# jianzongwu/DiffSensei

Measured on NVIDIA H100. Metric: unet_denoise_steps_per_sec_1024sq_bs4, higher is better.
Workload: dtype bf16

## Files before the change

### diffsensei_b200/csrc/attn_wgmma.cu

```cuda
#include <cstdlib>

#include "ds_common.cuh"
#include "ds_host.h"
#include "ip_mask.cuh"
#include "wgmma.cuh"

namespace ds {

constexpr int kQTile = 128;
constexpr int kKTile = 64;
constexpr int kHd = 64;
constexpr int kRing = 4;
constexpr int kAttnThreads = 384;
constexpr int kQBytes = kQTile * kHd * 2;
constexpr int kKVBytes = kKTile * kHd * 2;
constexpr int kAttnSmemBytes = kQBytes + kRing * 2 * kKVBytes + 1024  + 256 ;
constexpr float kLog2e = 1.4426950408889634f;

struct AttnParams {
  __nv_bfloat16* out;
  int Nq, ldo;
  int n_keys[2];
  int k_col0, v_col0;
  float scale_log2;
  const float* bbox;
  int num_ips, tokens_per_ip, num_dummy, Hd, Wd;
  float ip_scale;
};

__device__ __forceinline__ float ex2(float x) {
  float y;
  asm("ex2.approx.ftz.f32 %0, %1;" : "=f"(y) : "f"(x));
  return y;
}

__global__ void __launch_bounds__(kAttnThreads, 1)
attn_wgmma_kernel(const __grid_constant__ CUtensorMap tmQ, const __grid_constant__ CUtensorMap tmK0,
                  const __grid_constant__ CUtensorMap tmK1, const AttnParams p) {
  extern __shared__ uint8_t smem_raw[];
  const uint32_t raw_addr = smem_u32(smem_raw);
  uint8_t* smem = smem_raw + ((1024u - (raw_addr & 1023u)) & 1023u);
  uint8_t* sQ = smem;
  uint8_t* sRing = sQ + kQBytes;
  uint64_t* q_bar = reinterpret_cast<uint64_t*>(sRing + kRing * 2 * kKVBytes);
  uint64_t* full_bar = q_bar + 1;
  uint64_t* empty_bar = full_bar + kRing;

  const int warp = threadIdx.x >> 5, lane = threadIdx.x & 31;
  const int q0 = blockIdx.x * kQTile, head = blockIdx.y, b = blockIdx.z;
  const int tiles0 = (p.n_keys[0] + kKTile - 1) / kKTile;
  const int tiles1 = (p.n_keys[1] + kKTile - 1) / kKTile;

  if (warp == 0 && lane == 0) {
    tma_prefetch_desc(&tmQ);
    tma_prefetch_desc(&tmK0);
    if (tiles1 > 0) tma_prefetch_desc(&tmK1);
    mbar_init(q_bar, 1);
    for (int i = 0; i < kRing; ++i) {
      mbar_init(&full_bar[i], 1);
      mbar_init(&empty_bar[i], 256);
    }
    fence_mbar_init();
  }
  pdl_launch_dependents();
  __syncthreads();
  pdl_wait();

  if (warp < 4) {
    if (warp == 0 && lane == 0) {
      mbar_arrive_expect_tx(q_bar, kQBytes);
      tma_load_3d(sQ, &tmQ, q_bar, head * kHd, q0, b);
      int stage = 0;
      uint32_t phase = 0;
      for (int t = 0; t < tiles0 + tiles1; ++t) {
        const bool second = t >= tiles0;
        const CUtensorMap* m = second ? &tmK1 : &tmK0;
        const int key0 = (second ? t - tiles0 : t) * kKTile;
        mbar_wait(&empty_bar[stage], phase ^ 1);
        mbar_arrive_expect_tx(&full_bar[stage], 2 * kKVBytes);
        uint8_t* sK = sRing + stage * 2 * kKVBytes;
        tma_load_3d(sK, m, &full_bar[stage], p.k_col0 + head * kHd, key0, b);
        tma_load_3d(sK + kKVBytes, m, &full_bar[stage], p.v_col0 + head * kHd, key0, b);
        if (++stage == kRing) {
          stage = 0;
          phase ^= 1;
        }
      }
    }
    return;
  }

  const int ct = threadIdx.x - 128;
  const int wg = ct >> 7;
  const int r0 = (ct >> 5) * 16 + (lane >> 2);
  const int cq = 2 * (lane & 3);
  uint32_t ip_bits[2] = {0u, 0u};
  if (tiles1 > 0) {
    const float* bb = p.bbox + static_cast<size_t>(b) * p.num_ips * 4;
#pragma unroll
    for (int h = 0; h < 2; ++h) {
      const int n = q0 + r0 + 8 * h;
      if (n < p.Nq) ip_bits[h] = ip_inside_bits(bb, p.num_ips, n, p.Hd, p.Wd);
    }
  }
  const uint32_t q_addr = smem_u32(sQ) + wg * 64 * 128;
  mbar_wait(q_bar, 0);

  float o[32], res[32];
  float m_run[2], l_run[2];
  int stage = 0;
  uint32_t phase = 0;
  for (int set = 0; set < (tiles1 > 0 ? 2 : 1); ++set) {
    const int n_tiles = set ? tiles1 : tiles0;
    const int nk = set ? p.n_keys[1] : p.n_keys[0];
#pragma unroll
    for (int i = 0; i < 32; ++i) o[i] = 0.f;
    m_run[0] = m_run[1] = -INFINITY;
    l_run[0] = l_run[1] = 0.f;
    for (int t = 0; t < n_tiles; ++t) {
      mbar_wait(&full_bar[stage], phase);
      const uint32_t k_addr = smem_u32(sRing + stage * 2 * kKVBytes);
      const uint32_t v_addr = k_addr + kKVBytes;
      float s[32];
      wgmma_fence();
#pragma unroll
      for (int k = 0; k < kHd / 16; ++k)
        wgmma_m64n64_ss(s, make_wgmma_desc(q_addr + k * 32, 1024, 16), make_wgmma_desc(k_addr + k * 32, 1024, 16),
                        k != 0);
      wgmma_commit();
      wgmma_wait<0>();
      fence_regs<32>(s);

      const int key0 = t * kKTile;
      float mx[2] = {-INFINITY, -INFINITY};
#pragma unroll
      for (int j = 0; j < 8; ++j) {
#pragma unroll
        for (int e = 0; e < 4; ++e) {
          const int key = key0 + j * 8 + cq + (e & 1);
          const int h = e >> 1;
          float v = s[4 * j + e] * p.scale_log2;
          if (set == 1 && !ip_key_open(ip_bits[h], key, p.tokens_per_ip, p.num_dummy)) v -= 10000.0f * kLog2e;
          if (key >= nk) v = -INFINITY;
          s[4 * j + e] = v;
          mx[h] = fmaxf(mx[h], v);
        }
      }
      float corr[2];
#pragma unroll
      for (int h = 0; h < 2; ++h) {
        mx[h] = fmaxf(mx[h], __shfl_xor_sync(0xffffffffu, mx[h], 1));
        mx[h] = fmaxf(mx[h], __shfl_xor_sync(0xffffffffu, mx[h], 2));
        const float m_new = fmaxf(m_run[h], mx[h]);
        corr[h] = ex2(m_run[h] - m_new);
        m_run[h] = m_new;
        l_run[h] *= corr[h];
      }
      uint32_t pa[4][4];
#pragma unroll
      for (int j = 0; j < 8; ++j) {
#pragma unroll
        for (int h = 0; h < 2; ++h) {
          const float p0 = ex2(s[4 * j + 2 * h] - m_run[h]);
          const float p1 = ex2(s[4 * j + 2 * h + 1] - m_run[h]);
          l_run[h] += p0 + p1;
          pa[j >> 1][(j & 1) * 2 + h] = pack_bf16(p0, p1);
        }
      }
#pragma unroll
      for (int j = 0; j < 8; ++j) {
        o[4 * j + 0] *= corr[0];
        o[4 * j + 1] *= corr[0];
        o[4 * j + 2] *= corr[1];
        o[4 * j + 3] *= corr[1];
      }
      wgmma_fence();
#pragma unroll
      for (int kk = 0; kk < kKTile / 16; ++kk)
        wgmma_m64n64_rs_tb(o, pa[kk], make_wgmma_desc(v_addr + kk * 2048, 1024, 1024), 1);
      wgmma_commit();
      wgmma_wait<0>();
      fence_regs<32>(o);
      mbar_arrive(&empty_bar[stage]);
      if (++stage == kRing) {
        stage = 0;
        phase ^= 1;
      }
    }
#pragma unroll
    for (int h = 0; h < 2; ++h) {
      l_run[h] += __shfl_xor_sync(0xffffffffu, l_run[h], 1);
      l_run[h] += __shfl_xor_sync(0xffffffffu, l_run[h], 2);
    }
    const float w = set ? p.ip_scale : 1.0f;
    const float inv[2] = {w / l_run[0], w / l_run[1]};
#pragma unroll
    for (int i = 0; i < 32; ++i) {
      const float v = o[i] * inv[(i >> 1) & 1];
      res[i] = set ? res[i] + v : v;
    }
  }

#pragma unroll
  for (int h = 0; h < 2; ++h) {
    const int n = q0 + r0 + 8 * h;
    if (n >= p.Nq) continue;
    __nv_bfloat16* orow = p.out + (static_cast<size_t>(b) * p.Nq + n) * p.ldo + head * kHd + cq;
#pragma unroll
    for (int j = 0; j < 8; ++j)
      *reinterpret_cast<uint32_t*>(orow + j * 8) = pack_bf16(res[4 * j + 2 * h], res[4 * j + 2 * h + 1]);
  }
}

static bool make_tok_map(CUtensorMap* m, const void* base, int cols, int ld, int tokens, int batch, int box_rows) {
  const uint64_t dims[3] = {static_cast<uint64_t>(cols), static_cast<uint64_t>(tokens), static_cast<uint64_t>(batch)};
  const uint64_t strides[2] = {static_cast<uint64_t>(ld) * 2, static_cast<uint64_t>(tokens) * ld * 2};
  const uint32_t box[3] = {kHd, static_cast<uint32_t>(box_rows), 1};
  return encode_tmap_bf16(m, base, 3, dims, strides, box, nullptr);
}

static int launch_attn(const CUtensorMap& tmQ, const CUtensorMap& tmK0, const CUtensorMap& tmK1, const AttnParams& p,
                       int B, int heads, cudaStream_t st) {
  static bool attr_set[kMaxDevices] = {};
  bool& set = attr_set[device_slot()];
  if (!set) {
    DS_CUDA_OK(cudaFuncSetAttribute(attn_wgmma_kernel, cudaFuncAttributeMaxDynamicSharedMemorySize, kAttnSmemBytes));
    set = true;
  }
  cudaLaunchConfig_t cfg = {};
  cfg.gridDim = dim3((p.Nq + kQTile - 1) / kQTile, heads, B);
  cfg.blockDim = dim3(kAttnThreads);
  cfg.dynamicSmemBytes = kAttnSmemBytes;
  cfg.stream = st;
  cudaLaunchAttribute attr[1];
  pdl_attr(&attr[0]);
  cfg.attrs = attr;
  cfg.numAttrs = 1;
  DS_CUDA_OK(cudaLaunchKernelEx(&cfg, attn_wgmma_kernel, tmQ, tmK0, tmK1, p));
  DS_LAUNCH_OK("attn_wgmma_kernel");
  return DS_OK;
}

static int launch_flash(const void* q, int ldq, int q_cols, const void* kv, int ldkv, int kv_cols, int k_col0,
                        int v_col0, void* out, int ldo, int B, int Nq, int Nkv, int heads, float scale, cudaStream_t st) {
  DeviceInfo dev;
  if (!get_device(&dev)) return DS_ERR_CUDA;
  CUtensorMap tmQ, tmK;
  if (!make_tok_map(&tmQ, q, q_cols, ldq, Nq, B, kQTile)) return DS_ERR_CUDA;
  if (!make_tok_map(&tmK, kv, kv_cols, ldkv, Nkv, B, kKTile)) return DS_ERR_CUDA;
  AttnParams p{};
  p.out = static_cast<__nv_bfloat16*>(out);
  p.Nq = Nq;
  p.ldo = ldo;
  p.n_keys[0] = Nkv;
  p.n_keys[1] = 0;
  p.k_col0 = k_col0;
  p.v_col0 = v_col0;
  p.scale_log2 = scale * kLog2e;
  return launch_attn(tmQ, tmK, tmK, p, B, heads, st);
}

}

using namespace ds;

extern "C" int ds_attention_self(const void* qkv, void* out, int B, int N, int heads, void* stream) {
  DS_REQUIRE(qkv && out, "ds_attention_self: NULL pointer");
  DS_REQUIRE(B > 0 && N > 0 && heads > 0, "ds_attention_self: bad shape");
  DS_REQUIRE((reinterpret_cast<uintptr_t>(qkv) & 15) == 0 && (reinterpret_cast<uintptr_t>(out) & 15) == 0,
             "ds_attention_self: pointers must be 16-byte aligned");
  const int C = heads * kHd;
  return launch_flash(qkv, 3 * C, 3 * C, qkv, 3 * C, 3 * C, C, 2 * C, out, C, B, N, N, heads, 0.125f,
                      static_cast<cudaStream_t>(stream));
}

extern "C" int ds_resampler_attn(const void* q, const void* kv, void* out, int Bc, int nq, int n_kv, int heads,
                                 void* stream) {
  DS_REQUIRE(q && kv && out, "ds_resampler_attn: NULL pointer");
  DS_REQUIRE(Bc > 0 && nq > 0 && n_kv > 0 && heads > 0, "ds_resampler_attn: bad shape");
  DS_REQUIRE((reinterpret_cast<uintptr_t>(q) & 15) == 0 && (reinterpret_cast<uintptr_t>(kv) & 15) == 0 &&
                 (reinterpret_cast<uintptr_t>(out) & 15) == 0,
             "ds_resampler_attn: pointers must be 16-byte aligned");
  const int C = heads * kHd;
  return launch_flash(q, C, C, kv, 2 * C, 2 * C, 0, C, out, C, Bc, nq, n_kv, heads, 0.125f,
                      static_cast<cudaStream_t>(stream));
}

extern "C" int ds_attention_cross_ip(const ds_cross_ip_args* a, void* stream) {
  DS_REQUIRE(a != nullptr, "ds_attention_cross_ip: args is NULL");
  DS_REQUIRE(a->q && a->kv_text && a->kv_ip && a->bbox && a->out, "ds_attention_cross_ip: NULL pointer");
  DS_REQUIRE(a->B > 0 && a->N > 0 && a->heads > 0, "ds_attention_cross_ip: bad shape");
  DS_REQUIRE(a->n_text > 0 && a->n_ip > 0, "ds_attention_cross_ip: n_text and n_ip must be positive");
  DS_REQUIRE(a->num_ips > 0 && a->num_ips <= kMaxIps && a->tokens_per_ip > 0 && a->num_dummy >= 0 &&
                 a->num_dummy + a->num_ips * a->tokens_per_ip == a->n_ip,
             "ds_attention_cross_ip: n_ip (%d) != num_dummy (%d) + num_ips (%d) * tokens_per_ip (%d)", a->n_ip,
             a->num_dummy, a->num_ips, a->tokens_per_ip);
  DS_REQUIRE((reinterpret_cast<uintptr_t>(a->q) & 15) == 0 && (reinterpret_cast<uintptr_t>(a->kv_text) & 15) == 0 &&
                 (reinterpret_cast<uintptr_t>(a->kv_ip) & 15) == 0 && (reinterpret_cast<uintptr_t>(a->out) & 15) == 0,
             "ds_attention_cross_ip: pointers must be 16-byte aligned");
  int Hd, Wd;
  if (!derive_hw(a->N, a->aspect_ratio, &Hd, &Wd)) {
    set_error("ds_attention_cross_ip: cannot factor N=%d for aspect_ratio=%f", a->N, a->aspect_ratio);
    return DS_ERR_INVALID;
  }
  DeviceInfo dev;
  if (!get_device(&dev)) return DS_ERR_CUDA;
  const int C = a->heads * kHd;
  CUtensorMap tmQ, tmT, tmI;
  if (!make_tok_map(&tmQ, a->q, C, C, a->N, a->B, kQTile)) return DS_ERR_CUDA;
  if (!make_tok_map(&tmT, a->kv_text, 2 * C, 2 * C, a->n_text, a->B, kKTile)) return DS_ERR_CUDA;
  if (!make_tok_map(&tmI, a->kv_ip, 2 * C, 2 * C, a->n_ip, a->B, kKTile)) return DS_ERR_CUDA;
  AttnParams p{};
  p.out = static_cast<__nv_bfloat16*>(a->out);
  p.Nq = a->N;
  p.ldo = C;
  p.n_keys[0] = a->n_text;
  p.n_keys[1] = a->n_ip;
  p.k_col0 = 0;
  p.v_col0 = C;
  p.scale_log2 = 0.125f * kLog2e;
  p.bbox = a->bbox;
  p.num_ips = a->num_ips;
  p.tokens_per_ip = a->tokens_per_ip;
  p.num_dummy = a->num_dummy;
  p.Hd = Hd;
  p.Wd = Wd;
  p.ip_scale = a->ip_scale;
  return launch_attn(tmQ, tmT, tmI, p, a->B, a->heads, static_cast<cudaStream_t>(stream));
}
```

### diffsensei_b200/csrc/ip_mask.cuh

```cuda
#pragma once
#include <math.h>
#include <stdint.h>

namespace ds {

constexpr int kMaxIps = 16;

inline bool derive_hw(int N, double aspect_ratio, int* Hd, int* Wd) {
  if (N <= 0 || !(aspect_ratio > 0.0)) return false;
  long long width = static_cast<long long>(pow(static_cast<double>(N) / aspect_ratio, 0.5));
  if (width < 1) return false;
  long long height = N / width;
  while (width * height != N) {
    if (width * height < N)
      width += 1;
    else
      width -= 1;
    if (width < 1 || width > N) return false;
    height = N / width;
  }
  *Hd = static_cast<int>(height);
  *Wd = static_cast<int>(width);
  return true;
}

__device__ __forceinline__ float linspace01(int i, int steps) {
  if (steps <= 1) return 0.0f;
  const float step = __fdiv_rn(1.0f, static_cast<float>(steps - 1));
  return (i < steps / 2) ? __fmul_rn(step, static_cast<float>(i))
                         : __fmaf_rn(-step, static_cast<float>(steps - 1 - i), 1.0f);
}

__device__ __forceinline__ uint32_t ip_inside_bits(const float* __restrict__ bbox, int num_ips, int n, int Hd, int Wd) {
  const int yi = n / Wd, xi = n - yi * Wd;
  const float x = linspace01(xi, Wd), y = linspace01(yi, Hd);
  uint32_t bits = 0;
  for (int i = 0; i < num_ips; ++i) {
    const float x1 = bbox[4 * i], y1 = bbox[4 * i + 1], x2 = bbox[4 * i + 2], y2 = bbox[4 * i + 3];
    if (x >= x1 && x <= x2 && y >= y1 && y <= y2) bits |= 1u << i;
  }
  return bits;
}

__device__ __forceinline__ bool ip_key_open(uint32_t bits, int key, int tokens_per_ip, int num_dummy) {
  if (key < num_dummy) return bits == 0;
  return (bits >> ((key - num_dummy) / tokens_per_ip)) & 1u;
}

}
```

Baseline: 5.116.

## Pipeline QK/PV wgmma, add persistent resident-KV cross-attention kernel, rebalance registers

Restructures the attention loop so the next tile's QK^T wgmma is issued while the current tile's PV wgmma runs, overlapping softmax with tensor-core work. Adds setmaxnreg to shift registers from the producer warpgroup to the consumers. Adds a persistent cross-attention kernel that keeps the short text+IP KV resident in shared memory across query tiles and double-buffers Q loads. It also precomputes the IP mask as a 64-bit key bitmap and skips masking on full unmasked tiles. The pipelining raises register pressure and adds more complex synchronisation.

```diff
diff --git a/diffsensei_b200/csrc/attn_wgmma.cu b/diffsensei_b200/csrc/attn_wgmma.cu
--- a/diffsensei_b200/csrc/attn_wgmma.cu
+++ b/diffsensei_b200/csrc/attn_wgmma.cu
@@ -14,8 +14,13 @@
 constexpr int kAttnThreads = 384;
 constexpr int kQBytes = kQTile * kHd * 2;
 constexpr int kKVBytes = kKTile * kHd * 2;
-constexpr int kAttnSmemBytes = kQBytes + kRing * 2 * kKVBytes + 1024  + 256 ;
+constexpr int kStreamSmemBytes = kQBytes + kRing * 2 * kKVBytes + 1024  + 256 ;
+constexpr int kResidentTiles = 4;
+constexpr int kQBufs = 2;
+constexpr int kCrossSmemBytes = kResidentTiles * 2 * kKVBytes + kQBufs * kQBytes + 1024 + 256;
 constexpr float kLog2e = 1.4426950408889634f;
+constexpr int kProducerRegs = 40;
+constexpr int kConsumerRegs = 232;
 
 struct AttnParams {
   __nv_bfloat16* out;
@@ -26,6 +31,7 @@
   const float* bbox;
   int num_ips, tokens_per_ip, num_dummy, Hd, Wd;
   float ip_scale;
+  int heads, q_tiles, items;
 };
 
 __device__ __forceinline__ float ex2(float x) {
@@ -34,9 +40,205 @@
   return y;
 }
 
+struct SetMask {
+  int nk;
+  bool ip;
+  uint32_t ip_bits[2];
+  int tokens_per_ip, num_dummy;
+};
+
+__device__ __forceinline__ void issue_qk(float (&s)[32], uint32_t q_addr, uint32_t k_addr) {
+#pragma unroll
+  for (int k = 0; k < kHd / 16; ++k)
+    wgmma_m64n64_ss(s, make_wgmma_desc(q_addr + k * 32, 1024, 16), make_wgmma_desc(k_addr + k * 32, 1024, 16), k != 0);
+}
+
+__device__ __forceinline__ void issue_pv(float (&o)[32], const uint32_t (&pa)[4][4], uint32_t v_addr) {
+#pragma unroll
+  for (int kk = 0; kk < kKTile / 16; ++kk)
+    wgmma_m64n64_rs_tb(o, pa[kk], make_wgmma_desc(v_addr + kk * 2048, 1024, 1024), 1);
+}
+
+__device__ __forceinline__ void fence_operands(float (&o)[32], uint32_t (&pa)[4][4]) {
+  fence_regs<32>(o);
+#pragma unroll
+  for (int kk = 0; kk < 4; ++kk)
+#pragma unroll
+    for (int i = 0; i < 4; ++i) asm volatile("" : "+r"(pa[kk][i])::"memory");
+}
+
+template <bool kMasked>
+__device__ __forceinline__ void softmax_step(const float (&s)[32], int key0, const SetMask& mk,
+                                             const uint64_t (&open)[2], float scale_log2, int cq, float (&m_run)[2],
+                                             float (&l_run)[2], float (&corr)[2], uint32_t (&pa)[4][4]) {
+  float x[32];
+  float mx[2] = {-INFINITY, -INFINITY};
+#pragma unroll
+  for (int j = 0; j < 8; ++j) {
+#pragma unroll
+    for (int e = 0; e < 4; ++e) {
+      const int key = key0 + j * 8 + cq + (e & 1);
+      const int h = e >> 1;
+      float v = s[4 * j + e] * scale_log2;
+      if (kMasked) {
+        if (mk.ip && !((open[h] >> (j * 8 + (e & 1))) & 1u)) v -= 10000.0f * kLog2e;
+        if (key >= mk.nk) v = -INFINITY;
+      }
+      x[4 * j + e] = v;
+      mx[h] = fmaxf(mx[h], v);
+    }
+  }
+#pragma unroll
+  for (int h = 0; h < 2; ++h) {
+    mx[h] = fmaxf(mx[h], __shfl_xor_sync(0xffffffffu, mx[h], 1));
+    mx[h] = fmaxf(mx[h], __shfl_xor_sync(0xffffffffu, mx[h], 2));
+    const float m_new = fmaxf(m_run[h], mx[h]);
+    corr[h] = ex2(m_run[h] - m_new);
+    m_run[h] = m_new;
+    l_run[h] *= corr[h];
+  }
+#pragma unroll
+  for (int j = 0; j < 8; ++j) {
+#pragma unroll
+    for (int h = 0; h < 2; ++h) {
+      const float p0 = ex2(x[4 * j + 2 * h] - m_run[h]);
+      const float p1 = ex2(x[4 * j + 2 * h + 1] - m_run[h]);
+      l_run[h] += p0 + p1;
+      pa[j >> 1][(j & 1) * 2 + h] = pack_bf16(p0, p1);
+    }
+  }
+}
+
+__device__ __forceinline__ void softmax_tile(const float (&s)[32], int key0, const SetMask& mk, float scale_log2, int cq,
+                                             float (&m_run)[2], float (&l_run)[2], float (&corr)[2],
+                                             uint32_t (&pa)[4][4]) {
+  uint64_t open[2] = {0ull, 0ull};
+  if (mk.ip) {
+#pragma unroll
+    for (int h = 0; h < 2; ++h)
+      open[h] = ip_open_keys64(mk.ip_bits[h], key0, mk.tokens_per_ip, mk.num_dummy) >> cq;
+  }
+  if (mk.ip || key0 + kKTile > mk.nk)
+    softmax_step<true>(s, key0, mk, open, scale_log2, cq, m_run, l_run, corr, pa);
+  else
+    softmax_step<false>(s, key0, mk, open, scale_log2, cq, m_run, l_run, corr, pa);
+}
+
+template <class TileAddr, class Release>
+__device__ __forceinline__ void attend_set(float (&o)[32], float (&l_run)[2], uint32_t q_addr, int n_tiles,
+                                           const SetMask& mk, float scale_log2, int cq, TileAddr tile_addr,
+                                           Release release) {
+  float m_run[2] = {-INFINITY, -INFINITY};
+  l_run[0] = l_run[1] = 0.f;
+#pragma unroll
+  for (int i = 0; i < 32; ++i) o[i] = 0.f;
+  float s[32], corr[2];
+  uint32_t pa[4][4], pb[4][4];
+  uint32_t k_addr = tile_addr(0);
+  wgmma_fence();
+  issue_qk(s, q_addr, k_addr);
+  wgmma_commit();
+  wgmma_wait<0>();
+  fence_regs<32>(s);
+  softmax_tile(s, 0, mk, scale_log2, cq, m_run, l_run, corr, pa);
+
+  auto step = [&](int t, uint32_t(&cur)[4][4], uint32_t(&next)[4][4]) {
+    const uint32_t k_next = tile_addr(t + 1);
+    fence_operands(o, cur);
+    wgmma_fence();
+    issue_qk(s, q_addr, k_next);
+    wgmma_commit();
+    issue_pv(o, cur, k_addr + kKVBytes);
+    wgmma_commit();
+    wgmma_wait<1>();
+    fence_regs<32>(s);
+    softmax_tile(s, (t + 1) * kKTile, mk, scale_log2, cq, m_run, l_run, corr, next);
+    wgmma_wait<0>();
+    fence_regs<32>(o);
+    release(t);
+#pragma unroll
+    for (int j = 0; j < 8; ++j) {
+      o[4 * j + 0] *= corr[0];
+      o[4 * j + 1] *= corr[0];
+      o[4 * j + 2] *= corr[1];
+      o[4 * j + 3] *= corr[1];
+    }
+    k_addr = k_next;
+  };
+  auto last = [&](int t, uint32_t(&cur)[4][4]) {
+    fence_operands(o, cur);
+    wgmma_fence();
+    issue_pv(o, cur, k_addr + kKVBytes);
+    wgmma_commit();
+    wgmma_wait<0>();
+    fence_regs<32>(o);
+    release(t);
+  };
+  for (int t = 0;; t += 2) {
+    if (t + 1 == n_tiles) {
+      last(t, pa);
+      break;
+    }
+    step(t, pa, pb);
+    if (t + 2 == n_tiles) {
+      last(t + 1, pb);
+      break;
+    }
+    step(t + 1, pb, pa);
+  }
+}
+
+__device__ __forceinline__ void normalise_into(float (&res)[32], const float (&o)[32], float (&l_run)[2], float w,
+                                               bool accumulate) {
+#pragma unroll
+  for (int h = 0; h < 2; ++h) {
+    l_run[h] += __shfl_xor_sync(0xffffffffu, l_run[h], 1);
+    l_run[h] += __shfl_xor_sync(0xffffffffu, l_run[h], 2);
+  }
+  const float inv[2] = {w / l_run[0], w / l_run[1]};
+#pragma unroll
+  for (int i = 0; i < 32; ++i) {
+    const float v = o[i] * inv[(i >> 1) & 1];
+    res[i] = accumulate ? res[i] + v : v;
+  }
+}
+
+__device__ __forceinline__ void store_rows(const AttnParams& p, const float (&res)[32], int b, int head, int row0,
+                                           int cq) {
+#pragma unroll
+  for (int h = 0; h < 2; ++h) {
+    const int n = row0 + 8 * h;
+    if (n >= p.Nq) continue;
+    __nv_bfloat16* orow = p.out + (static_cast<size_t>(b) * p.Nq + n) * p.ldo + head * kHd + cq;
+#pragma unroll
+    for (int j = 0; j < 8; ++j)
+      *reinterpret_cast<uint32_t*>(orow + j * 8) = pack_bf16(res[4 * j + 2 * h], res[4 * j + 2 * h + 1]);
+  }
+}
+
+__device__ __forceinline__ void ip_row_bits(const AttnParams& p, int b, int row0, uint32_t (&bits)[2]) {
+  const float* bb = p.bbox + static_cast<size_t>(b) * p.num_ips * 4;
+#pragma unroll
+  for (int h = 0; h < 2; ++h) {
+    const int n = row0 + 8 * h;
+    bits[h] = n < p.Nq ? ip_inside_bits(bb, p.num_ips, n, p.Hd, p.Wd) : 0u;
+  }
+}
+
+__device__ __forceinline__ SetMask set_mask(const AttnParams& p, int set, const uint32_t (&bits)[2]) {
+  SetMask mk;
+  mk.nk = set ? p.n_keys[1] : p.n_keys[0];
+  mk.ip = set == 1;
+  mk.ip_bits[0] = bits[0];
+  mk.ip_bits[1] = bits[1];
+  mk.tokens_per_ip = p.tokens_per_ip;
+  mk.num_dummy = p.num_dummy;
+  return mk;
+}
+
 __global__ void __launch_bounds__(kAttnThreads, 1)
-attn_wgmma_kernel(const __grid_constant__ CUtensorMap tmQ, const __grid_constant__ CUtensorMap tmK0,
-                  const __grid_constant__ CUtensorMap tmK1, const AttnParams p) {
+attn_stream_kernel(const __grid_constant__ CUtensorMap tmQ, const __grid_constant__ CUtensorMap tmK0,
+                   const __grid_constant__ CUtensorMap tmK1, const AttnParams p) {
   extern __shared__ uint8_t smem_raw[];
   const uint32_t raw_addr = smem_u32(smem_raw);
   uint8_t* smem = smem_raw + ((1024u - (raw_addr & 1023u)) & 1023u);
@@ -67,6 +269,7 @@
   pdl_wait();
 
   if (warp < 4) {
+    setmaxnreg_dec<kProducerRegs>();
     if (warp == 0 && lane == 0) {
       mbar_arrive_expect_tx(q_bar, kQBytes);
       tma_load_3d(sQ, &tmQ, q_bar, head * kHd, q0, b);
@@ -90,125 +293,142 @@
     return;
   }
 
+  setmaxnreg_inc<kConsumerRegs>();
   const int ct = threadIdx.x - 128;
   const int wg = ct >> 7;
   const int r0 = (ct >> 5) * 16 + (lane >> 2);
   const int cq = 2 * (lane & 3);
   uint32_t ip_bits[2] = {0u, 0u};
-  if (tiles1 > 0) {
-    const float* bb = p.bbox + static_cast<size_t>(b) * p.num_ips * 4;
-#pragma unroll
-    for (int h = 0; h < 2; ++h) {
-      const int n = q0 + r0 + 8 * h;
-      if (n < p.Nq) ip_bits[h] = ip_inside_bits(bb, p.num_ips, n, p.Hd, p.Wd);
-    }
-  }
+  if (tiles1 > 0) ip_row_bits(p, b, q0 + r0, ip_bits);
   const uint32_t q_addr = smem_u32(sQ) + wg * 64 * 128;
+  const uint32_t ring_addr = smem_u32(sRing);
   mbar_wait(q_bar, 0);
 
-  float o[32], res[32];
-  float m_run[2], l_run[2];
+  float o[32], res[32], l_run[2];
   int stage = 0;
   uint32_t phase = 0;
+  auto tile_addr = [&](int) {
+    mbar_wait(&full_bar[stage], phase);
+    const uint32_t a = ring_addr + stage * 2 * kKVBytes;
+    if (++stage == kRing) {
+      stage = 0;
+      phase ^= 1;
+    }
+    return a;
+  };
+  int rstage = 0;
+  auto release = [&](int) {
+    mbar_arrive(&empty_bar[rstage]);
+    if (++rstage == kRing) rstage = 0;
+  };
   for (int set = 0; set < (tiles1 > 0 ? 2 : 1); ++set) {
-    const int n_tiles = set ? tiles1 : tiles0;
-    const int nk = set ? p.n_keys[1] : p.n_keys[0];
-#pragma unroll
-    for (int i = 0; i < 32; ++i) o[i] = 0.f;
-    m_run[0] = m_run[1] = -INFINITY;
-    l_run[0] = l_run[1] = 0.f;
-    for (int t = 0; t < n_tiles; ++t) {
-      mbar_wait(&full_bar[stage], phase);
-      const uint32_t k_addr = smem_u32(sRing + stage * 2 * kKVBytes);
-      const uint32_t v_addr = k_addr + kKVBytes;
-      float s[32];
-      wgmma_fence();
-#pragma unroll
-      for (int k = 0; k < kHd / 16; ++k)
-        wgmma_m64n64_ss(s, make_wgmma_desc(q_addr + k * 32, 1024, 16), make_wgmma_desc(k_addr + k * 32, 1024, 16),
-                        k != 0);
-      wgmma_commit();
-      wgmma_wait<0>();
-      fence_regs<32>(s);
-
-      const int key0 = t * kKTile;
-      float mx[2] = {-INFINITY, -INFINITY};
-#pragma unroll
-      for (int j = 0; j < 8; ++j) {
-#pragma unroll
-        for (int e = 0; e < 4; ++e) {
-          const int key = key0 + j * 8 + cq + (e & 1);
-          const int h = e >> 1;
-          float v = s[4 * j + e] * p.scale_log2;
-          if (set == 1 && !ip_key_open(ip_bits[h], key, p.tokens_per_ip, p.num_dummy)) v -= 10000.0f * kLog2e;
-          if (key >= nk) v = -INFINITY;
-          s[4 * j + e] = v;
-          mx[h] = fmaxf(mx[h], v);
+    const SetMask mk = set_mask(p, set, ip_bits);
+    attend_set(o, l_run, q_addr, set ? tiles1 : tiles0, mk, p.scale_log2, cq, tile_addr, release);
+    normalise_into(res, o, l_run, set ? p.ip_scale : 1.0f, set != 0);
+  }
+  store_rows(p, res, b, head, q0 + r0, cq);
+}
+
+__global__ void __launch_bounds__(kAttnThreads, 1)
+attn_cross_kernel(const __grid_constant__ CUtensorMap tmQ, const __grid_constant__ CUtensorMap tmK0,
+                  const __grid_constant__ CUtensorMap tmK1, const AttnParams p) {
+  extern __shared__ uint8_t smem_raw[];
+  const uint32_t raw_addr = smem_u32(smem_raw);
+  uint8_t* smem = smem_raw + ((1024u - (raw_addr & 1023u)) & 1023u);
+  uint8_t* sKV = smem;
+  uint8_t* sQ = sKV + kResidentTiles * 2 * kKVBytes;
+  uint64_t* kv_full = reinterpret_cast<uint64_t*>(sQ + kQBufs * kQBytes);
+  uint64_t* kv_empty = kv_full + 1;
+  uint64_t* q_full = kv_empty + 1;
+  uint64_t* q_empty = q_full + kQBufs;
+
+  const int warp = threadIdx.x >> 5, lane = threadIdx.x & 31;
+  const int tiles0 = (p.n_keys[0] + kKTile - 1) / kKTile;
+  const int tiles1 = (p.n_keys[1] + kKTile - 1) / kKTile;
+  const int item_lo = static_cast<int>(static_cast<long long>(blockIdx.x) * p.items / gridDim.x);
+  const int item_hi = static_cast<int>(static_cast<long long>(blockIdx.x + 1) * p.items / gridDim.x);
+
+  if (warp == 0 && lane == 0) {
+    tma_prefetch_desc(&tmQ);
+    tma_prefetch_desc(&tmK0);
+    tma_prefetch_desc(&tmK1);
+    mbar_init(kv_full, 1);
+    mbar_init(kv_empty, 256);
+    for (int i = 0; i < kQBufs; ++i) {
+      mbar_init(&q_full[i], 1);
+      mbar_init(&q_empty[i], 256);
+    }
+    fence_mbar_init();
+  }
+  pdl_launch_dependents();
+  __syncthreads();
+  pdl_wait();
+
+  if (warp < 4) {
+    setmaxnreg_dec<kProducerRegs>();
+    if (warp == 0 && lane == 0) {
+      int pair = -1;
+      uint32_t kv_phase = 0;
+      for (int item = item_lo, it = 0; item < item_hi; ++item, ++it) {
+        const int ip = item / p.q_tiles, qt = item - ip * p.q_tiles;
+        const int b = ip / p.heads, head = ip - b * p.heads;
+        if (ip != pair) {
+          pair = ip;
+          mbar_wait(kv_empty, kv_phase ^ 1);
+          kv_phase ^= 1;
+          mbar_arrive_expect_tx(kv_full, (tiles0 + tiles1) * 2 * kKVBytes);
+          for (int t = 0; t < tiles0 + tiles1; ++t) {
+            const bool second = t >= tiles0;
+            const CUtensorMap* m = second ? &tmK1 : &tmK0;
+            const int key0 = (second ? t - tiles0 : t) * kKTile;
+            uint8_t* sK = sKV + t * 2 * kKVBytes;
+            tma_load_3d(sK, m, kv_full, p.k_col0 + head * kHd, key0, b);
+            tma_load_3d(sK + kKVBytes, m, kv_full, p.v_col0 + head * kHd, key0, b);
+          }
         }
+        const int buf = it & 1;
+        mbar_wait(&q_empty[buf], ((it >> 1) & 1) ^ 1);
+        mbar_arrive_expect_tx(&q_full[buf], kQBytes);
+        tma_load_3d(sQ + buf * kQBytes, &tmQ, &q_full[buf], head * kHd, qt * kQTile, b);
       }
-      float corr[2];
-#pragma unroll
-      for (int h = 0; h < 2; ++h) {
-        mx[h] = fmaxf(mx[h], __shfl_xor_sync(0xffffffffu, mx[h], 1));
-        mx[h] = fmaxf(mx[h], __shfl_xor_sync(0xffffffffu, mx[h], 2));
-        const float m_new = fmaxf(m_run[h], mx[h]);
-        corr[h] = ex2(m_run[h] - m_new);
-        m_run[h] = m_new;
-        l_run[h] *= corr[h];
-      }
-      uint32_t pa[4][4];
-#pragma unroll
-      for (int j = 0; j < 8; ++j) {
-#pragma unroll
-        for (int h = 0; h < 2; ++h) {
-          const float p0 = ex2(s[4 * j + 2 * h] - m_run[h]);
-          const float p1 = ex2(s[4 * j + 2 * h + 1] - m_run[h]);
-          l_run[h] += p0 + p1;
-          pa[j >> 1][(j & 1) * 2 + h] = pack_bf16(p0, p1);
-        }
-      }
-#pragma unroll
-      for (int j = 0; j < 8; ++j) {
-        o[4 * j + 0] *= corr[0];
-        o[4 * j + 1] *= corr[0];
-        o[4 * j + 2] *= corr[1];
-        o[4 * j + 3] *= corr[1];
-      }
-      wgmma_fence();
-#pragma unroll
-      for (int kk = 0; kk < kKTile / 16; ++kk)
-        wgmma_m64n64_rs_tb(o, pa[kk], make_wgmma_desc(v_addr + kk * 2048, 1024, 1024), 1);
-      wgmma_commit();
-      wgmma_wait<0>();
-      fence_regs<32>(o);
-      mbar_arrive(&empty_bar[stage]);
-      if (++stage == kRing) {
-        stage = 0;
-        phase ^= 1;
-      }
-    }
-#pragma unroll
-    for (int h = 0; h < 2; ++h) {
-      l_run[h] += __shfl_xor_sync(0xffffffffu, l_run[h], 1);
-      l_run[h] += __shfl_xor_sync(0xffffffffu, l_run[h], 2);
-    }
-    const float w = set ? p.ip_scale : 1.0f;
-    const float inv[2] = {w / l_run[0], w / l_run[1]};
-#pragma unroll
-    for (int i = 0; i < 32; ++i) {
-      const float v = o[i] * inv[(i >> 1) & 1];
-      res[i] = set ? res[i] + v : v;
-    }
-  }
-
-#pragma unroll
-  for (int h = 0; h < 2; ++h) {
-    const int n = q0 + r0 + 8 * h;
-    if (n >= p.Nq) continue;
-    __nv_bfloat16* orow = p.out + (static_cast<size_t>(b) * p.Nq + n) * p.ldo + head * kHd + cq;
-#pragma unroll
-    for (int j = 0; j < 8; ++j)
-      *reinterpret_cast<uint32_t*>(orow + j * 8) = pack_bf16(res[4 * j + 2 * h], res[4 * j + 2 * h + 1]);
+    }
+    return;
+  }
+
+  setmaxnreg_inc<kConsumerRegs>();
+  const int ct = threadIdx.x - 128;
+  const int wg = ct >> 7;
+  const int r0 = (ct >> 5) * 16 + (lane >> 2);
+  const int cq = 2 * (lane & 3);
+  const uint32_t kv_addr = smem_u32(sKV);
+  const uint32_t q_base = smem_u32(sQ) + wg * 64 * 128;
+  int pair = -1;
+  uint32_t kv_phase = 0;
+  for (int item = item_lo, it = 0; item < item_hi; ++item, ++it) {
+    const int ip = item / p.q_tiles, qt = item - ip * p.q_tiles;
+    const int b = ip / p.heads, head = ip - b * p.heads;
+    const int q0 = qt * kQTile;
+    if (ip != pair) {
+      if (pair >= 0) mbar_arrive(kv_empty);
+      pair = ip;
+      mbar_wait(kv_full, kv_phase);
+      kv_phase ^= 1;
+    }
+    uint32_t ip_bits[2];
+    ip_row_bits(p, b, q0 + r0, ip_bits);
+    const int buf = it & 1;
+    const uint32_t q_addr = q_base + buf * kQBytes;
+    mbar_wait(&q_full[buf], (it >> 1) & 1);
+    float o[32], res[32], l_run[2];
+    for (int set = 0; set < 2; ++set) {
+      const SetMask mk = set_mask(p, set, ip_bits);
+      const uint32_t set_addr = kv_addr + (set ? tiles0 : 0) * 2 * kKVBytes;
+      attend_set(o, l_run, q_addr, set ? tiles1 : tiles0, mk, p.scale_log2, cq,
+                 [&](int t) { return set_addr + t * 2 * kKVBytes; }, [](int) {});
+      normalise_into(res, o, l_run, set ? p.ip_scale : 1.0f, set != 0);
+    }
+    mbar_arrive(&q_empty[buf]);
+    store_rows(p, res, b, head, q0 + r0, cq);
   }
 }
 
@@ -219,26 +439,35 @@
   return encode_tmap_bf16(m, base, 3, dims, strides, box, nullptr);
 }
 
-static int launch_attn(const CUtensorMap& tmQ, const CUtensorMap& tmK0, const CUtensorMap& tmK1, const AttnParams& p,
-                       int B, int heads, cudaStream_t st) {
-  static bool attr_set[kMaxDevices] = {};
+using AttnKernel = void (*)(CUtensorMap, CUtensorMap, CUtensorMap, AttnParams);
+
+static int launch_attn(AttnKernel kernel, const char* name, int smem_bytes, bool* attr_set, dim3 grid,
+                       const CUtensorMap& tmQ, const CUtensorMap& tmK0, const CUtensorMap& tmK1, const AttnParams& p,
+                       cudaStream_t st) {
   bool& set = attr_set[device_slot()];
   if (!set) {
-    DS_CUDA_OK(cudaFuncSetAttribute(attn_wgmma_kernel, cudaFuncAttributeMaxDynamicSharedMemorySize, kAttnSmemBytes));
+    DS_CUDA_OK(cudaFuncSetAttribute(kernel, cudaFuncAttributeMaxDynamicSharedMemorySize, smem_bytes));
     set = true;
   }
   cudaLaunchConfig_t cfg = {};
-  cfg.gridDim = dim3((p.Nq + kQTile - 1) / kQTile, heads, B);
+  cfg.gridDim = grid;
   cfg.blockDim = dim3(kAttnThreads);
-  cfg.dynamicSmemBytes = kAttnSmemBytes;
+  cfg.dynamicSmemBytes = smem_bytes;
   cfg.stream = st;
   cudaLaunchAttribute attr[1];
   pdl_attr(&attr[0]);
   cfg.attrs = attr;
   cfg.numAttrs = 1;
-  DS_CUDA_OK(cudaLaunchKernelEx(&cfg, attn_wgmma_kernel, tmQ, tmK0, tmK1, p));
-  DS_LAUNCH_OK("attn_wgmma_kernel");
+  DS_CUDA_OK(cudaLaunchKernelEx(&cfg, kernel, tmQ, tmK0, tmK1, p));
+  DS_LAUNCH_OK(name);
   return DS_OK;
+}
+
+static int launch_stream(const CUtensorMap& tmQ, const CUtensorMap& tmK0, const CUtensorMap& tmK1,
+                         const AttnParams& p, int B, int heads, cudaStream_t st) {
+  static bool attr_set[kMaxDevices] = {};
+  return launch_attn(attn_stream_kernel, "attn_stream_kernel", kStreamSmemBytes, attr_set,
+                     dim3((p.Nq + kQTile - 1) / kQTile, heads, B), tmQ, tmK0, tmK1, p, st);
 }
 
 static int launch_flash(const void* q, int ldq, int q_cols, const void* kv, int ldkv, int kv_cols, int k_col0,
@@ -257,7 +486,7 @@
   p.k_col0 = k_col0;
   p.v_col0 = v_col0;
   p.scale_log2 = scale * kLog2e;
-  return launch_attn(tmQ, tmK, tmK, p, B, heads, st);
+  return launch_stream(tmQ, tmK, tmK, p, B, heads, st);
 }
 
 }
@@ -326,5 +555,16 @@
   p.Hd = Hd;
   p.Wd = Wd;
   p.ip_scale = a->ip_scale;
-  return launch_attn(tmQ, tmT, tmI, p, a->B, a->heads, static_cast<cudaStream_t>(stream));
-}
+  cudaStream_t st = static_cast<cudaStream_t>(stream);
+  const int tiles = (a->n_text + kKTile - 1) / kKTile + (a->n_ip + kKTile - 1) / kKTile;
+  if (tiles > kResidentTiles) return launch_stream(tmQ, tmT, tmI, p, a->B, a->heads, st);
+  p.heads = a->heads;
+  p.q_tiles = (a->N + kQTile - 1) / kQTile;
+  const long long items = static_cast<long long>(a->B) * a->heads * p.q_tiles;
+  DS_REQUIRE(items <= INT32_MAX, "ds_attention_cross_ip: too many query tiles");
+  p.items = static_cast<int>(items);
+  const int ctas = static_cast<int>(items < dev.num_sms ? items : dev.num_sms);
+  static bool attr_set[kMaxDevices] = {};
+  return launch_attn(attn_cross_kernel, "attn_cross_kernel", kCrossSmemBytes, attr_set, dim3(ctas), tmQ, tmT, tmI,
+                     p, st);
+}
diff --git a/diffsensei_b200/csrc/ip_mask.cuh b/diffsensei_b200/csrc/ip_mask.cuh
--- a/diffsensei_b200/csrc/ip_mask.cuh
+++ b/diffsensei_b200/csrc/ip_mask.cuh
@@ -47,4 +47,21 @@
   return (bits >> ((key - num_dummy) / tokens_per_ip)) & 1u;
 }
 
+__device__ __forceinline__ uint64_t bit_range64(int lo, int hi) {
+  lo = max(lo, 0);
+  hi = min(hi, 64);
+  if (lo >= hi) return 0ull;
+  const uint64_t below_hi = hi == 64 ? ~0ull : (1ull << hi) - 1ull;
+  return below_hi & ~((1ull << lo) - 1ull);
 }
+
+__device__ __forceinline__ uint64_t ip_open_keys64(uint32_t bits, int key0, int tokens_per_ip, int num_dummy) {
+  uint64_t m = bits == 0 ? bit_range64(-key0, num_dummy - key0) : 0ull;
+  for (uint32_t r = bits; r != 0; r &= r - 1) {
+    const int lo = num_dummy + (__ffs(r) - 1) * tokens_per_ip - key0;
+    m |= bit_range64(lo, lo + tokens_per_ip);
+  }
+  return m;
+}
+
+}
```

New measurement: 6.172 (median of 6 runs). 1.21x the previous value.
